# Prashant-ambati/Federated-Learning-for-Privacy-Preserving-Image-Classification

Hardware: AMD Instinct MI355X
Metric: client-images/sec/node (higher is better)
Workload: dtype f32; 1 GPU; KT: cifar10_cnn 32 clients (32/GPU), non_iid(a=0.5), 1 local epoch(s), batch 32, sgd lr 0.01, DP eps=None, FedAvg; clients=32, images_per_round=45015, batch=32, parallelism=client-packed x1 GPU

## Files before the change

### federated-learning-for-privacy-preserving-image-classification_amd/csrc/layers.hip

```cpp
#include "fh_common.h"

namespace fh {

typedef float hf32x4 __attribute__((ext_vector_type(4)));

__global__ void __launch_bounds__(256)
maxpool2_fwd_kernel(const float* __restrict__ x, int64_t x_cs, float* __restrict__ y,
                    int64_t y_cs, uint8_t* __restrict__ idx, int64_t i_cs,
                    uint8_t* __restrict__ mask, int64_t m_cs, const int32_t* __restrict__ counts,
                    int batch, int C, int H, int W, int drop_mode, float keep_prob, float scale,
                    uint64_t seed_salt, const uint64_t* __restrict__ seed_dev,
                    const float* __restrict__ in_scale, const float* __restrict__ in_shift,
                    int64_t aff_cs, int xh, int xw, int yh, int yw) {
    const uint64_t seed = seed_salt + (seed_dev ? *seed_dev : 0ull);
    const int z = blockIdx.y;
    const uint64_t prow = drop_mode == 1 ? philox_row(seed_dev, z) : 0ull;
    const int cnt = counts ? counts[z] : batch;
    const int OH = H / 2, OW = W / 2;
    const uint32_t per_img = (uint32_t)(C * OH * OW);
    const uint32_t total = (uint32_t)cnt * per_img;
    const float* xb = x + z * x_cs;
    for (uint32_t e = blockIdx.x * blockDim.x + threadIdx.x; e < total;
         e += gridDim.x * blockDim.x) {
        const uint32_t t = e / (uint32_t)OW;
        const int ow = (int)(e - t * (uint32_t)OW);
        const uint32_t plane = t / (uint32_t)OH;
        const int oh = (int)(t - plane * (uint32_t)OH);
        const float* p = xb + (int64_t)plane * xh * xw + (2 * oh) * xw + 2 * ow;
        float v0 = p[0], v1 = p[1], v2 = p[xw], v3 = p[xw + 1];
        if (in_scale) {
            const int c = (int)(plane % C);
            const float s = in_scale[z * aff_cs + c], t = in_shift[z * aff_cs + c];
            v0 = fmaxf(v0 * s + t, 0.f);
            v1 = fmaxf(v1 * s + t, 0.f);
            v2 = fmaxf(v2 * s + t, 0.f);
            v3 = fmaxf(v3 * s + t, 0.f);
        }
        float m = v0;
        int a = 0;
        if (v1 > m) { m = v1; a = 1; }
        if (v2 > m) { m = v2; a = 2; }
        if (v3 > m) { m = v3; a = 3; }
        idx[z * i_cs + e] = (uint8_t)a;
        if (drop_mode) {
            uint8_t keep;
            if (drop_mode == 1) {
                const uint4 r = Philox::gen(seed, prow, (uint64_t)e);
                keep = u01(r.x) <= keep_prob ? 1 : 0;
                mask[z * m_cs + e] = keep;
            } else {
                keep = mask[z * m_cs + e];
            }
            m = keep ? m * scale : 0.f;
        }
        y[z * y_cs + (int64_t)plane * yh * yw + oh * yw + ow] = m;
    }
}

__global__ void __launch_bounds__(256)
maxpool2_bwd_kernel(const float* __restrict__ dy, int64_t dy_cs, const uint8_t* __restrict__ idx,
                    int64_t i_cs, const uint8_t* __restrict__ mask, int64_t m_cs,
                    const float* __restrict__ xin, int64_t x_cs, float* __restrict__ dx,
                    int64_t dx_cs, const int32_t* __restrict__ counts, int batch, int C, int H,
                    int W, float scale, int gh, int gw, int xh, int xw,
                    const float* __restrict__ yin, int64_t yin_cs) {
    const int z = blockIdx.y;
    const int cnt = counts ? counts[z] : batch;
    const int OH = H / 2, OW = W / 2;
    const uint32_t total = (uint32_t)cnt * (uint32_t)(C * OH * OW);
    for (uint32_t e = blockIdx.x * blockDim.x + threadIdx.x; e < total;
         e += gridDim.x * blockDim.x) {
        const uint32_t t = e / (uint32_t)OW;
        const int ow = (int)(e - t * (uint32_t)OW);
        const uint32_t pl = t / (uint32_t)OH;
        const int oh = (int)(t - pl * (uint32_t)OH);
        const int64_t plane = pl;
        float g = dy[z * dy_cs + plane * gh * gw + oh * gw + ow];
        if (mask) g = mask[z * m_cs + e] ? g * scale : 0.f;
        const int a = idx[z * i_cs + e];
        const int64_t base = plane * xh * xw + (2 * oh) * xw + 2 * ow;
        const int64_t off[4] = {0, 1, xw, xw + 1};
        if (xin && !(xin[z * x_cs + base + off[a]] > 0.f)) g = 0.f;
        if (yin && !(yin[z * yin_cs + plane * gh * gw + oh * gw + ow] > 0.f)) g = 0.f;
        float* d = dx + z * dx_cs + base;
#pragma unroll
        for (int q = 0; q < 4; ++q) d[off[q]] = (q == a) ? g : 0.f;
    }
}

__global__ void __launch_bounds__(256)
dropout_fwd_kernel(const float* __restrict__ x, int64_t x_cs, float* __restrict__ y, int64_t y_cs,
                   uint8_t* __restrict__ mask, int64_t m_cs, const int32_t* __restrict__ counts,
                   int batch, int64_t per_img, int drop_mode, float keep_prob, float scale,
                   uint64_t seed_salt, const uint64_t* __restrict__ seed_dev) {
    const uint64_t seed = seed_salt + (seed_dev ? *seed_dev : 0ull);
    const int z = blockIdx.y;
    const uint64_t prow = drop_mode == 1 ? philox_row(seed_dev, z) : 0ull;
    const int cnt = counts ? counts[z] : batch;
    const int64_t total = cnt * per_img;
    for (int64_t e = blockIdx.x * (int64_t)blockDim.x + threadIdx.x; e < total;
         e += (int64_t)gridDim.x * blockDim.x) {
        uint8_t keep;
        if (drop_mode == 1) {
            const uint4 r = Philox::gen(seed, prow, (uint64_t)e);
            keep = u01(r.x) <= keep_prob ? 1 : 0;
            mask[z * m_cs + e] = keep;
        } else {
            keep = mask[z * m_cs + e];
        }
        const float v = x[z * x_cs + e];
        y[z * y_cs + e] = keep ? v * scale : 0.f;
    }
}

__global__ void __launch_bounds__(256)
dropout_bwd_kernel(const float* __restrict__ dy, int64_t dy_cs, const uint8_t* __restrict__ mask,
                   int64_t m_cs, const float* __restrict__ relu_out, int64_t r_cs,
                   float* __restrict__ dx, int64_t dx_cs, const int32_t* __restrict__ counts,
                   int batch, int64_t per_img, float scale) {
    const int z = blockIdx.y;
    const int cnt = counts ? counts[z] : batch;
    const int64_t total = cnt * per_img;
    for (int64_t e = blockIdx.x * (int64_t)blockDim.x + threadIdx.x; e < total;
         e += (int64_t)gridDim.x * blockDim.x) {
        float g = dy[z * dy_cs + e];
        if (mask) g = mask[z * m_cs + e] ? g * scale : 0.f;
        if (relu_out && !(relu_out[z * r_cs + e] > 0.f)) g = 0.f;
        dx[z * dx_cs + e] = g;
    }
}

__global__ void __launch_bounds__(256)
ce_kernel(const float* __restrict__ logits, int64_t l_cs, const int64_t* __restrict__ targets,
          int64_t t_cs, float* __restrict__ dlogits, int64_t d_cs, float* __restrict__ loss_out,
          double* __restrict__ acc_loss, int64_t* __restrict__ acc_correct,
          int64_t* __restrict__ acc_seen, const int32_t* __restrict__ reset,
          const int32_t* __restrict__ counts, int batch, int K) {
    __shared__ double sl[4];
    __shared__ int sc[4];
    __shared__ double li[256];
    __shared__ int ci[256];
    const int z = blockIdx.x;
    const int cnt = counts ? counts[z] : batch;
    const int lane = threadIdx.x & 63, wid = threadIdx.x >> 6;
    double lsum = 0.0;
    int corr = 0;
    const float inv_n = cnt > 0 ? 1.0f / (float)cnt : 0.f;
    if (K <= 16 && cnt <= 256) {
        const int g = threadIdx.x >> 4, l = threadIdx.x & 15;
        for (int img = g; img < cnt; img += 16) {
            const float* row = logits + z * l_cs + (int64_t)img * K;
            const int tgt = (int)targets[z * t_cs + img];
            const float v = l < K ? row[l] : -INFINITY;
            float mx = v;
            int amax = l < K ? l : K;
#pragma unroll
            for (int o = 8; o > 0; o >>= 1) {
                const float om = __shfl_xor(mx, o, 16);
                const int oa = __shfl_xor(amax, o, 16);
                if (om > mx || (om == mx && oa < amax)) { mx = om; amax = oa; }
            }
            float se = l < K ? expf(v - mx) : 0.f;
#pragma unroll
            for (int o = 8; o > 0; o >>= 1) se += __shfl_xor(se, o, 16);
            const float lse = logf(se);
            if (l == 0) {
                li[img] = (double)(-((row[tgt] - mx) - lse));
                ci[img] = amax == tgt;
            }
            if (l < K) {
                const float p = expf((v - mx) - lse);
                dlogits[z * d_cs + (int64_t)img * K + l] = (p - (l == tgt ? 1.f : 0.f)) * inv_n;
            }
        }
        __syncthreads();
        if (threadIdx.x < 4) {
            for (int img = threadIdx.x; img < cnt; img += 4) {
                lsum += li[img];
                corr += ci[img];
            }
            sl[threadIdx.x] = lsum;
            sc[threadIdx.x] = corr;
        }
        __syncthreads();
        if (threadIdx.x == 0) {
            const double tot = sl[0] + sl[1] + sl[2] + sl[3];
            const float batch_loss = cnt > 0 ? (float)(tot / (double)cnt) : 0.f;
            const bool rs = reset && reset[z];
            if (loss_out) loss_out[z] = batch_loss;
            if (acc_loss) acc_loss[z] = (rs ? 0.0 : acc_loss[z]) + (double)batch_loss;
            if (acc_correct) acc_correct[z] = (rs ? 0 : acc_correct[z]) + sc[0] + sc[1] + sc[2] + sc[3];
            if (acc_seen) acc_seen[z] = (rs ? 0 : acc_seen[z]) + cnt;
        }
        return;
    }
    for (int img = wid; img < cnt; img += 4) {
        const float* row = logits + z * l_cs + (int64_t)img * K;
        const int tgt = (int)targets[z * t_cs + img];
        float mx = -INFINITY;
        int amax = 0;
        for (int k = lane; k < K; k += 64) {
            const float v = row[k];
            if (v > mx) { mx = v; amax = k; }
        }
#pragma unroll
        for (int o = 32; o > 0; o >>= 1) {
            const float om = __shfl_xor(mx, o, 64);
            const int oa = __shfl_xor(amax, o, 64);
            if (om > mx || (om == mx && oa < amax)) { mx = om; amax = oa; }
        }
        float se = 0.f;
        for (int k = lane; k < K; k += 64) se += expf(row[k] - mx);
        se = wave_sum(se);
        const float lse = logf(se);
        if (lane == 0) {
            lsum += (double)(-((row[tgt] - mx) - lse));
            corr += (amax == tgt);
        }
        float* drow = dlogits + z * d_cs + (int64_t)img * K;
        for (int k = lane; k < K; k += 64) {
            const float p = expf((row[k] - mx) - lse);
            drow[k] = (p - (k == tgt ? 1.f : 0.f)) * inv_n;
        }
    }
    if (lane == 0) {
        sl[wid] = lsum;
        sc[wid] = corr;
    }
    __syncthreads();
    if (threadIdx.x == 0) {
        const double tot = sl[0] + sl[1] + sl[2] + sl[3];
        const float batch_loss = cnt > 0 ? (float)(tot / (double)cnt) : 0.f;
        const bool rs = reset && reset[z];
        if (loss_out) loss_out[z] = batch_loss;
        if (acc_loss) acc_loss[z] = (rs ? 0.0 : acc_loss[z]) + (double)batch_loss;
        if (acc_correct) acc_correct[z] = (rs ? 0 : acc_correct[z]) + sc[0] + sc[1] + sc[2] + sc[3];
        if (acc_seen) acc_seen[z] = (rs ? 0 : acc_seen[z]) + cnt;
    }
}

constexpr int kHeadBlocks = 4;
template <bool SMALLK>
__global__ void __launch_bounds__(256)
linear_head_ce_kernel(const float* __restrict__ x, int64_t x_cs, const float* __restrict__ w,
                      int64_t w_cs, const float* __restrict__ bias, int64_t b_cs,
                      const int64_t* __restrict__ targets, int64_t t_cs, float* __restrict__ logits,
                      int64_t l_cs, float* __restrict__ dlogits, int64_t d_cs,
                      float* __restrict__ loss_out, double* __restrict__ acc_loss,
                      int64_t* __restrict__ acc_correct, int64_t* __restrict__ acc_seen,
                      const int32_t* __restrict__ reset, float* __restrict__ dw, int64_t dw_cs,
                      float* __restrict__ db, int64_t db_cs, float* __restrict__ dx,
                      int64_t dx_cs, const uint8_t* __restrict__ mask, int64_t m_cs, float scale,
                      int relu_in, const int32_t* __restrict__ counts, int batch, int F, int K) {
    constexpr int KMAX = SMALLK ? 16 : 128;
    constexpr int FMAX = 256;
    constexpr int XS = SMALLK ? 32 * (FMAX + 1) : 1;
    constexpr int WS = SMALLK ? KMAX * (FMAX + 1) : 1;
    __shared__ float Xs[XS];
    __shared__ float Ws[WS];
    __shared__ float L[32 * KMAX];
    __shared__ float D[32 * KMAX];
    __shared__ double li[32];
    __shared__ int ci[32];
    __shared__ double sl[4];
    __shared__ int sc[4];
    constexpr int MS = SMALLK ? 32 * FMAX : 1;
    __shared__ int64_t Ts[32];
    __shared__ float Bs[KMAX];
    __shared__ uint8_t Ms[MS];
    const int z = blockIdx.y, part = blockIdx.x, tid = threadIdx.x;
    const int cnt = counts ? counts[z] : batch;
    const float* xz = x + z * x_cs;
    const float* wz = w + z * w_cs;
    const int FP = F + 1;
    const int S = gridDim.x;
    bool rs0 = false;
    double al0 = 0.0;
    int64_t ac0 = 0, as0 = 0;
    auto load_acc = [&]() {
        if (part == 0 && tid == 0) {
            rs0 = reset && reset[z];
            if (acc_loss) al0 = acc_loss[z];
            if (acc_correct) ac0 = acc_correct[z];
            if (acc_seen) as0 = acc_seen[z];
        }
    };
    const int dx_per = (cnt * F + S - 1) / S, dx_e0 = part * dx_per;
    const int dx_e1 = min(cnt * F, dx_e0 + dx_per);
    if constexpr (SMALLK) {
        const int64_t tv = tid < cnt ? targets[z * t_cs + tid] : 0;
        const float bv = (tid < K && bias) ? bias[z * b_cs + tid] : 0.f;
        const uint8_t* mz = mask + z * m_cs;
        const bool mwords = mask && dx && ((uintptr_t)mz & 3) == 0;
        constexpr int NM = 32 * FMAX / 4 / 256;
        uint32_t mw[NM];
        if (mwords) {
#pragma unroll
            for (int i = 0; i < NM; ++i) {
                const int e = tid + 256 * i;
                mw[i] = e < cnt * F / 4 ? reinterpret_cast<const uint32_t*>(mz)[e] : 0u;
            }
        }
        const bool v4 = (F & 3) == 0 && ((uintptr_t)xz & 15) == 0 && ((uintptr_t)wz & 15) == 0;
        constexpr int NX = 32 * FMAX / 4 / 256, NW = KMAX * FMAX / 4 / 256;
        const int F4 = F / 4;
        float4 xv[NX], wv[NW];
        if (v4) {
#pragma unroll
            for (int i = 0; i < NX; ++i) {
                const int e4 = tid + 256 * i;
                xv[i] = e4 < cnt * F4 ? *reinterpret_cast<const float4*>(xz + 4 * e4)
                                      : make_float4(0.f, 0.f, 0.f, 0.f);
            }
#pragma unroll
            for (int i = 0; i < NW; ++i) {
                const int e4 = tid + 256 * i;
                wv[i] = e4 < K * F4 ? *reinterpret_cast<const float4*>(wz + 4 * e4)
                                    : make_float4(0.f, 0.f, 0.f, 0.f);
            }
        }
        load_acc();
        if (tid < cnt) Ts[tid] = tv;
        if (tid < K) Bs[tid] = bv;
        if (mwords) {
#pragma unroll
            for (int i = 0; i < NM; ++i) {
                const int e = tid + 256 * i;
                if (e < cnt * F / 4) reinterpret_cast<uint32_t*>(Ms)[e] = mw[i];
            }
        } else if (mask && dx) {
            for (int e = tid; e < cnt * F; e += 256) Ms[e] = mz[e];
        }
        if (v4) {
#pragma unroll
            for (int i = 0; i < NX; ++i) {
                const int e4 = tid + 256 * i;
                if (e4 < cnt * F4) {
                    const int b = e4 / F4, f = 4 * (e4 - b * F4);
                    float* d = Xs + b * FP + f;
                    d[0] = xv[i].x; d[1] = xv[i].y; d[2] = xv[i].z; d[3] = xv[i].w;
                }
            }
#pragma unroll
            for (int i = 0; i < NW; ++i) {
                const int e4 = tid + 256 * i;
                if (e4 < K * F4) {
                    const int k = e4 / F4, f = 4 * (e4 - k * F4);
                    float* d = Ws + k * FP + f;
                    d[0] = wv[i].x; d[1] = wv[i].y; d[2] = wv[i].z; d[3] = wv[i].w;
                }
            }
        } else {
            for (int e = tid; e < cnt * F; e += 256) {
                const int b = e / F;
                Xs[b * FP + (e - b * F)] = xz[e];
            }
            for (int e = tid; e < K * F; e += 256) {
                const int k = e / F;
                Ws[k * FP + (e - k * F)] = wz[e];
            }
        }
        __syncthreads();
    } else {
        load_acc();
    }
    auto X = [&](int b, int f) -> float { return SMALLK ? Xs[b * FP + f] : xz[(int64_t)b * F + f]; };
    auto Wt = [&](int k, int f) -> float { return SMALLK ? Ws[k * FP + f] : wz[(int64_t)k * F + f]; };
    const int lane = tid & 63, wid = tid >> 6;
    if constexpr (SMALLK) {
        const int mn = lane & 15, kk = lane >> 4, t = wid & 1, fh = wid >> 1, Fh = F >> 1;
        const int ia = t * 16 + mn;
        const bool arow = ia < cnt, bcol = mn < K;
        const float* xa = Xs + ia * FP + fh * Fh + kk;
        const float* wb = Ws + mn * FP + fh * Fh + kk;
        constexpr int NQ = FMAX / 8;
        float xr[NQ], wr[NQ];
#pragma unroll
        for (int u = 0; u < NQ; ++u) {
            const float xv = xa[4 * u], wv2 = wb[4 * u];
            xr[u] = arow ? xv : 0.f;
            wr[u] = bcol ? wv2 : 0.f;
        }
        hf32x4 acc = {0.f, 0.f, 0.f, 0.f};
#pragma unroll
        for (int u = 0; u < NQ; ++u)
            if (4 * u < Fh) acc = __builtin_amdgcn_mfma_f32_16x16x4f32(xr[u], wr[u], acc, 0, 0, 0);
        float* lp = fh ? D : L;
#pragma unroll
        for (int r = 0; r < 4; ++r) lp[(t * 16 + 4 * kk + r) * 16 + mn] = acc[r];
        __syncthreads();
        float lv[2];
#pragma unroll
        for (int u = 0; u < 2; ++u) {
            const int o = tid + 256 * u;
            const int img = o / K, k = o - img * K;
            lv[u] = o < cnt * K ? L[img * 16 + k] + D[img * 16 + k] : 0.f;
        }
        __syncthreads();
#pragma unroll
        for (int u = 0; u < 2; ++u) {
            const int o = tid + 256 * u;
            if (o < cnt * K) L[o] = bias ? lv[u] + Bs[o - (o / K) * K] : lv[u];
        }
    } else {
        for (int o = tid; o < cnt * K; o += 256) {
            const int img = o / K, k = o - img * K;
            float a0 = 0.f, a1 = 0.f, a2 = 0.f, a3 = 0.f;
            for (int f = 0; f < F; f += 4) {
                a0 = fmaf(X(img, f), Wt(k, f), a0);
                a1 = fmaf(X(img, f + 1), Wt(k, f + 1), a1);
                a2 = fmaf(X(img, f + 2), Wt(k, f + 2), a2);
                a3 = fmaf(X(img, f + 3), Wt(k, f + 3), a3);
            }
            const float acc = (a0 + a1) + (a2 + a3);
            L[img * K + k] = bias ? acc + bias[z * b_cs + k] : acc;
        }
    }
    __syncthreads();
    const float inv_n = cnt > 0 ? 1.0f / (float)cnt : 0.f;
    double lsum = 0.0;
    int corr = 0;
    if (K <= 16) {
        const int g = tid >> 4, l = tid & 15;
        float v[2], mx[2], se[2];
        int amax[2], tgt[2];
#pragma unroll
        for (int u = 0; u < 2; ++u) {
            const int img = g + 16 * u;
            tgt[u] = img < cnt ? (SMALLK ? (int)Ts[img] : (int)targets[z * t_cs + img]) : 0;
            v[u] = l < K ? L[img * K + l] : -INFINITY;
            mx[u] = v[u];
            amax[u] = l < K ? l : K;
        }
#pragma unroll
        for (int o = 8; o > 0; o >>= 1)
#pragma unroll
            for (int u = 0; u < 2; ++u) {
                const float om = __shfl_xor(mx[u], o, 16);
                const int oa = __shfl_xor(amax[u], o, 16);
                if (om > mx[u] || (om == mx[u] && oa < amax[u])) { mx[u] = om; amax[u] = oa; }
            }
#pragma unroll
        for (int u = 0; u < 2; ++u) se[u] = l < K ? expf(v[u] - mx[u]) : 0.f;
#pragma unroll
        for (int o = 8; o > 0; o >>= 1)
#pragma unroll
            for (int u = 0; u < 2; ++u) se[u] += __shfl_xor(se[u], o, 16);
#pragma unroll
        for (int u = 0; u < 2; ++u) {
            const int img = g + 16 * u;
            if (img >= cnt) break;
            const float lse = logf(se[u]);
            if (l == 0) {
                li[img] = (double)(-((L[img * K + tgt[u]] - mx[u]) - lse));
                ci[img] = amax[u] == tgt[u];
            }
            if (l < K) {
                const float p = expf((v[u] - mx[u]) - lse);
                D[img * K + l] = (p - (l == tgt[u] ? 1.f : 0.f)) * inv_n;
            }
        }
        __syncthreads();
        if (tid < 4) {
            double lv[8];
            int cv[8];
#pragma unroll
            for (int j = 0; j < 8; ++j) {
                lv[j] = li[tid + 4 * j];
                cv[j] = ci[tid + 4 * j];
            }
#pragma unroll
            for (int j = 0; j < 8; ++j)
                if (tid + 4 * j < cnt) {
                    lsum += lv[j];
                    corr += cv[j];
                }
            sl[tid] = lsum;
            sc[tid] = corr;
        }
    } else {
        for (int img = wid; img < cnt; img += 4) {
            const float* row = L + img * K;
            const int tgt = (int)targets[z * t_cs + img];
            float mx = -INFINITY;
            int amax = 0;
            for (int k = lane; k < K; k += 64) {
                const float v = row[k];
                if (v > mx) { mx = v; amax = k; }
            }
#pragma unroll
            for (int o = 32; o > 0; o >>= 1) {
                const float om = __shfl_xor(mx, o, 64);
                const int oa = __shfl_xor(amax, o, 64);
                if (om > mx || (om == mx && oa < amax)) { mx = om; amax = oa; }
            }
            float se = 0.f;
            for (int k = lane; k < K; k += 64) se += expf(row[k] - mx);
            se = wave_sum(se);
            const float lse = logf(se);
            if (lane == 0) {
                lsum += (double)(-((row[tgt] - mx) - lse));
                corr += (amax == tgt);
            }
            for (int k = lane; k < K; k += 64) {
                const float p = expf((row[k] - mx) - lse);
                D[img * K + k] = (p - (k == tgt ? 1.f : 0.f)) * inv_n;
            }
        }
        if (lane == 0) {
            sl[wid] = lsum;
            sc[wid] = corr;
        }
    }
    __syncthreads();
    if (part == 0) {
        if (tid == 0) {
            const double tot = sl[0] + sl[1] + sl[2] + sl[3];
            const float batch_loss = cnt > 0 ? (float)(tot / (double)cnt) : 0.f;
            if (loss_out) loss_out[z] = batch_loss;
            if (acc_loss) acc_loss[z] = (rs0 ? 0.0 : al0) + (double)batch_loss;
            if (acc_correct) acc_correct[z] = (rs0 ? 0 : ac0) + sc[0] + sc[1] + sc[2] + sc[3];
            if (acc_seen) acc_seen[z] = (rs0 ? 0 : as0) + cnt;
        }
        for (int o = tid; o < cnt * K; o += 256) {
            logits[z * l_cs + o] = L[o];
            dlogits[z * d_cs + o] = D[o];
        }
        if (SMALLK && db && wid == 0) {
            const int k = lane & 15, g = lane >> 4;
            float v = 0.f, dv[8];
#pragma unroll
            for (int j = 0; j < 8; ++j) dv[j] = D[(g + 4 * j) * K + k];
            if (k < K)
#pragma unroll
                for (int j = 0; j < 8; ++j)
                    if (g + 4 * j < cnt) v += dv[j];
            v += __shfl_xor(v, 16, 64);
            v += __shfl_xor(v, 32, 64);
            if (lane < K) db[z * db_cs + lane] = v;
        } else if (db && tid < K) {
            float v = 0.f;
            for (int b = 0; b < cnt; ++b) v += D[b * K + tid];
            db[z * db_cs + tid] = v;
        }
    }
    if (SMALLK && dw) {
        const int mn = lane & 15, kk = lane >> 4;
        for (int tt = part + S * wid; tt < F / 16; tt += 4 * S) {
            const int f0 = tt * 16;
            float dr[8], xr2[8];
#pragma unroll
            for (int q = 0; q < 8; ++q) {
                const int b = 4 * q + kk;
                const bool ok = b < cnt;
                const float dv = D[b * K + mn], xv = Xs[b * FP + f0 + mn];
                dr[q] = ok && mn < K ? dv : 0.f;
                xr2[q] = ok ? xv : 0.f;
            }
            hf32x4 acc = {0.f, 0.f, 0.f, 0.f};
#pragma unroll
            for (int q = 0; q < 8; ++q)
                if (4 * q < cnt) acc = __builtin_amdgcn_mfma_f32_16x16x4f32(dr[q], xr2[q], acc, 0, 0, 0);
#pragma unroll
            for (int r = 0; r < 4; ++r) {
                const int k = 4 * kk + r;
                if (k < K) dw[z * dw_cs + (int64_t)k * F + f0 + mn] = acc[r];
            }
        }
    } else if (dw) {
        const int per = (K * F + S - 1) / S, e0 = part * per, e1 = min(K * F, e0 + per);
        for (int e = e0 + tid; e < e1; e += 256) {
            const int k = e / F, f = e - k * F;
            float a0 = 0.f, a1 = 0.f;
            int b = 0;
            for (; b + 1 < cnt; b += 2) {
                a0 = fmaf(D[b * K + k], X(b, f), a0);
                a1 = fmaf(D[(b + 1) * K + k], X(b + 1, f), a1);
            }
            if (b < cnt) a0 = fmaf(D[b * K + k], X(b, f), a0);
            dw[z * dw_cs + e] = a0 + a1;
        }
    }
    if (SMALLK && dx) {
        const int mn = lane & 15, kk = lane >> 4;
        for (int tt = part + S * wid; tt < 2 * (F / 16); tt += 4 * S) {
            const int t = tt & 1, f0 = (tt >> 1) * 16;
            if (t * 16 >= cnt) continue;
            const int ia = t * 16 + mn;
            float dr[KMAX / 4], wr2[KMAX / 4];
#pragma unroll
            for (int q = 0; q < KMAX / 4; ++q) {
                const int k = 4 * q + kk;
                const float dv = D[ia * K + k], wv2 = Ws[k * FP + f0 + mn];
                dr[q] = k < K && ia < cnt ? dv : 0.f;
                wr2[q] = k < K ? wv2 : 0.f;
            }
            hf32x4 acc = {0.f, 0.f, 0.f, 0.f};
#pragma unroll
            for (int q = 0; q < KMAX / 4; ++q)
                if (4 * q < K) acc = __builtin_amdgcn_mfma_f32_16x16x4f32(dr[q], wr2[q], acc, 0, 0, 0);
#pragma unroll
            for (int r = 0; r < 4; ++r) {
                const int img = t * 16 + 4 * kk + r, f = f0 + mn;
                if (img < cnt) {
                    float v = acc[r];
                    if (mask) v = Ms[img * F + f] ? v * scale : 0.f;
                    if (relu_in && !(Xs[img * FP + f] > 0.f)) v = 0.f;
                    dx[z * dx_cs + (int64_t)img * F + f] = v;
                }
            }
        }
    } else if (dx) {
        const int e0 = dx_e0, e1 = dx_e1;
        for (int eb = e0 + tid; eb < e1; eb += 4 * 256) {
            uint8_t mk[4];
#pragma unroll
            for (int u = 0; u < 4; ++u) {
                const int e = eb + 256 * u;
                mk[u] = (mask && e < e1) ? mask[z * m_cs + e] : 1;
            }
#pragma unroll
            for (int u = 0; u < 4; ++u) {
                const int e = eb + 256 * u;
                if (e >= e1) break;
                const int img = e / F, f = e - img * F;
                float acc = 0.f;
                for (int k = 0; k < K; ++k) acc = fmaf(D[img * K + k], Wt(k, f), acc);
                if (mask) acc = mk[u] ? acc * scale : 0.f;
                if (relu_in && !(X(img, f) > 0.f)) acc = 0.f;
                dx[z * dx_cs + e] = acc;
            }
        }
    }
}

__global__ void __launch_bounds__(256)
eval_metrics_kernel(const float* __restrict__ logits, int64_t l_cs,
                    const int64_t* __restrict__ targets, int64_t t_cs,
                    const int32_t* __restrict__ counts, int batch, int K,
                    double* __restrict__ loss_sum, int64_t* __restrict__ correct,
                    unsigned long long* __restrict__ class_correct,
                    unsigned long long* __restrict__ class_total) {
    __shared__ double sl[4];
    __shared__ int sc[4];
    const int z = blockIdx.x;
    const int cnt = counts ? counts[z] : batch;
    const int lane = threadIdx.x & 63, wid = threadIdx.x >> 6;
    double lsum = 0.0;
    int corr = 0;
    for (int img = wid; img < cnt; img += 4) {
        const float* row = logits + z * l_cs + (int64_t)img * K;
        const int tgt = (int)targets[z * t_cs + img];
        float mx = -INFINITY;
        int amax = 0;
        for (int k = lane; k < K; k += 64) {
            const float v = row[k];
            if (v > mx) { mx = v; amax = k; }
        }
#pragma unroll
        for (int o = 32; o > 0; o >>= 1) {
            const float om = __shfl_xor(mx, o, 64);
            const int oa = __shfl_xor(amax, o, 64);
            if (om > mx || (om == mx && oa < amax)) { mx = om; amax = oa; }
        }
        float se = 0.f;
        for (int k = lane; k < K; k += 64) se += expf(row[k] - mx);
        se = wave_sum(se);
        if (lane == 0) {
            lsum += (double)(-((row[tgt] - mx) - logf(se)));
            const int hit = amax == tgt;
            corr += hit;
            if (class_total && tgt >= 0 && tgt < K) {
                atomicAdd(class_total + tgt, 1ull);
                if (hit) atomicAdd(class_correct + tgt, 1ull);
            }
        }
    }
    if (lane == 0) {
        sl[wid] = lsum;
        sc[wid] = corr;
    }
    __syncthreads();
    if (threadIdx.x == 0) {
        if (loss_sum) loss_sum[z] += sl[0] + sl[1] + sl[2] + sl[3];
        if (correct) correct[z] += sc[0] + sc[1] + sc[2] + sc[3];
    }
}

__global__ void __launch_bounds__(256)
avgpool_fwd_kernel(const float* __restrict__ x, int64_t x_cs, float* __restrict__ y, int64_t y_cs,
                   const int32_t* __restrict__ counts, int batch, int C, int HW) {
    const int z = blockIdx.y;
    const int cnt = counts ? counts[z] : batch;
    const int lane = threadIdx.x & 63;
    const int64_t planes = (int64_t)cnt * C;
    for (int64_t pl = blockIdx.x * 4 + (threadIdx.x >> 6); pl < planes; pl += gridDim.x * 4) {
        const float* b = x + z * x_cs + pl * HW;
        float s = 0.f;
        for (int p = lane; p < HW; p += 64) s += b[p];
        s = wave_sum(s);
        if (lane == 0) y[z * y_cs + pl] = s / (float)HW;
    }
}

__global__ void __launch_bounds__(256)
avgpool_bwd_kernel(const float* __restrict__ dy, int64_t dy_cs, float* __restrict__ dx,
                   int64_t dx_cs, const int32_t* __restrict__ counts, int batch, int C, int HW) {
    const int z = blockIdx.y;
    const int cnt = counts ? counts[z] : batch;
    const int64_t total = (int64_t)cnt * C * HW;
    const float inv = 1.0f / (float)HW;
    for (int64_t e = blockIdx.x * (int64_t)blockDim.x + threadIdx.x; e < total;
         e += (int64_t)gridDim.x * blockDim.x)
        dx[z * dx_cs + e] = dy[z * dy_cs + e / HW] * inv;
}

__global__ void __launch_bounds__(256)
gather_kernel(const float* __restrict__ data, const int64_t* __restrict__ labels,
              const int64_t* __restrict__ idx, int64_t idx_cs, float* __restrict__ x, int64_t x_cs,
              int64_t* __restrict__ y, int64_t y_cs, int64_t sample_elems,
              const int32_t* __restrict__ counts, int batch) {
    const int z = blockIdx.y;
    const int cnt = counts ? counts[z] : batch;
    const int64_t total = (int64_t)cnt * sample_elems;
    constexpr int U = 4;
    const int64_t G = (int64_t)gridDim.x * blockDim.x;
    for (int64_t e0 = blockIdx.x * (int64_t)blockDim.x + threadIdx.x; e0 < total; e0 += U * G) {
        int64_t bq[U], oq[U], sq[U];
        float v[U];
#pragma unroll
        for (int u = 0; u < U; ++u) {
            const int64_t e = e0 + u * G;
            bq[u] = e < total ? e / sample_elems : 0;
            oq[u] = e - bq[u] * sample_elems;
            sq[u] = e < total ? idx[z * idx_cs + bq[u]] : 0;
        }
#pragma unroll
        for (int u = 0; u < U; ++u)
            v[u] = e0 + u * G < total ? data[sq[u] * sample_elems + oq[u]] : 0.f;
#pragma unroll
        for (int u = 0; u < U; ++u) {
            const int64_t e = e0 + u * G;
            if (e >= total) break;
            x[z * x_cs + e] = v[u];
            if (oq[u] == 0 && y) y[z * y_cs + bq[u]] = labels[sq[u]];
        }
    }
}

struct NormParams {
    float mean[4];
    float stdv[4];
};

__global__ void __launch_bounds__(256)
gather_u8_kernel(const uint8_t* __restrict__ data, const int64_t* __restrict__ labels,
                 const int64_t* __restrict__ idx, int64_t idx_cs, float* __restrict__ x,
                 int64_t x_cs, int64_t* __restrict__ y, int64_t y_cs,
                 const int32_t* __restrict__ counts, int batch, int C, int H, int W,
                 NormParams np, int pad, int flip, const uchar4* __restrict__ aug_in,
                 uchar4* __restrict__ aug_out, int64_t aug_cs, uint64_t seed_salt,
                 const uint64_t* __restrict__ seed_dev) {
    const int z = blockIdx.y;
    const int cnt = counts ? counts[z] : batch;
    const uint32_t plane = (uint32_t)(H * W), per = plane * (uint32_t)C;
    const uint32_t total = (uint32_t)cnt * per;
    const uint64_t seed = seed_salt + (seed_dev ? *seed_dev : 0ull);
    const uint64_t prow = philox_row(seed_dev, z);
    constexpr int U = 4;
    const uint32_t G = gridDim.x * blockDim.x;
    const bool aug = pad > 0 || flip;
    for (uint32_t e0 = blockIdx.x * blockDim.x + threadIdx.x; e0 < total; e0 += U * G) {
        uint32_t bq[U], rq[U];
        int cq[U], sy[U], sx[U];
        int64_t sq[U];
        uchar4 aq[U];
#pragma unroll
        for (int u = 0; u < U; ++u) {
            const uint32_t e = e0 + u * G;
            const uint32_t b = e < total ? e / per : 0u;
            bq[u] = b;
            rq[u] = e - b * per;
            sq[u] = idx[z * idx_cs + b];
            aq[u] = aug_in ? aug_in[z * aug_cs + b] : make_uchar4(0, 0, 0, 0);
        }
#pragma unroll
        for (int u = 0; u < U; ++u) {
            const uint32_t e = e0 + u * G, b = bq[u], r = rq[u];
            const int c = (int)(r / plane);
            const uint32_t p = r - (uint32_t)c * plane;
            const int yy = (int)(p / (uint32_t)W), xx = (int)(p - (uint32_t)yy * (uint32_t)W);
            int ci = pad, cj = pad, fl = 0;
            if (e < total && aug) {
                if (aug_in) {
                    ci = aq[u].x; cj = aq[u].y; fl = aq[u].z;
                } else {
                    const uint4 rr = Philox::gen(seed, prow, (uint64_t)b);
                    const uint32_t span = 2u * (uint32_t)pad + 1u;
                    ci = pad > 0 ? (int)(((uint64_t)rr.x * span) >> 32) : 0;
                    cj = pad > 0 ? (int)(((uint64_t)rr.y * span) >> 32) : 0;
                    fl = flip ? (int)(rr.z >> 31) : 0;
                    if (aug_out && r == 0) aug_out[z * aug_cs + b] = make_uchar4(ci, cj, fl, 0);
                }
            }
            const int sx0 = fl ? (W - 1 - xx) : xx;
            cq[u] = c;
            sy[u] = yy + ci - pad;
            sx[u] = sx0 + cj - pad;
        }
        uint32_t ub[U];
        int64_t lq[U];
        bool inq[U];
#pragma unroll
        for (int u = 0; u < U; ++u) {
            inq[u] = e0 + u * G < total && sy[u] >= 0 && sy[u] < H && sx[u] >= 0 && sx[u] < W;
            const int64_t off = inq[u] ? ((sq[u] * H + sy[u]) * W + sx[u]) * C + cq[u] : 0;
            ub[u] = data[off];
            lq[u] = labels[sq[u]];
        }
#pragma unroll
        for (int u = 0; u < U; ++u) {
            const uint32_t e = e0 + u * G;
            if (e >= total) break;
            const float v = __fdiv_rn(inq[u] ? (float)ub[u] : 0.f, 255.f);
            x[z * x_cs + e] = __fdiv_rn(v - np.mean[cq[u]], np.stdv[cq[u]]);
            if (rq[u] == 0 && y) y[z * y_cs + bq[u]] = lq[u];
        }
    }
}

static int ew_grid(int64_t n) { return (int)std::min<int64_t>(std::max<int64_t>(ceil_div(n, 256), 1), 2048); }

}

using namespace fh;

static int maxpool2_fwd_impl(const float* x, int64_t x_cs, const float* in_scale,
                             const float* in_shift, int64_t aff_cs, float* y, int64_t y_cs,
                             uint8_t* idx, int64_t i_cs, uint8_t* mask, int64_t m_cs,
                             const int32_t* counts, int32_t nclients, int32_t batch, int32_t C,
                             int32_t H, int32_t W, int32_t drop_mode, float p_drop, uint64_t seed,
                             const uint64_t* seed_dev, void* stream, int32_t xh = 0,
                             int32_t xw = 0, int32_t yh = 0, int32_t yw = 0) {
    if (xh == 0) { xh = H; xw = W; yh = H / 2; yw = W / 2; }
    FH_REQUIRE(nclients >= 0 && batch > 0 && C > 0 && H >= 2 && W >= 2, "maxpool2_fwd: bad shape");
    FH_REQUIRE(xh >= H && xw >= W && yh >= H / 2 && yw >= W / 2, "maxpool2_fwd: plane %dx%d / "
               "%dx%d smaller than the map %dx%d", xh, xw, yh, yw, H, W);
    FH_REQUIRE((H % 2) == 0 && (W % 2) == 0, "maxpool2_fwd: odd spatial size %dx%d", H, W);
    FH_REQUIRE(drop_mode >= 0 && drop_mode <= 2 && (drop_mode == 0 || mask), "maxpool2_fwd: mask");
    FH_REQUIRE(p_drop >= 0.f && p_drop < 1.f, "maxpool2_fwd: p=%g", p_drop);
    if (nclients == 0) return FH_OK;
    FH_REQUIRE(x && y && idx, "maxpool2_fwd: null pointer");
    const float keep = 1.0f - p_drop, scale = 1.0f / keep;
    const int64_t per = (int64_t)batch * C * (H / 2) * (W / 2);
    FH_LAUNCH(maxpool2_fwd_kernel, dim3(ew_grid(per), nclients), dim3(256), 0,
                       as_stream(stream), x, x_cs, y, y_cs, idx, i_cs, mask, m_cs, counts, batch, C,
                       H, W, drop_mode, keep, scale, seed, seed_dev, in_scale, in_shift, aff_cs,
                       xh, xw, yh, yw);
    FH_LAUNCH_CHECK("maxpool2_fwd");
    return FH_OK;
}

extern "C" int fh_maxpool2_fwd(const float* x, int64_t x_cs, float* y, int64_t y_cs, uint8_t* idx,
                               int64_t i_cs, uint8_t* mask, int64_t m_cs, const int32_t* counts,
                               int32_t nclients, int32_t batch, int32_t C, int32_t H, int32_t W,
                               int32_t drop_mode, float p_drop, uint64_t seed,
                               const uint64_t* seed_dev, void* stream) {
    return maxpool2_fwd_impl(x, x_cs, nullptr, nullptr, 0, y, y_cs, idx, i_cs, mask, m_cs, counts,
                             nclients, batch, C, H, W, drop_mode, p_drop, seed, seed_dev, stream);
}

extern "C" int fh_maxpool2_fwd_bnrelu(const float* x, int64_t x_cs, const float* in_scale,
                                      const float* in_shift, int64_t aff_cs, float* y,
                                      int64_t y_cs, uint8_t* idx, int64_t i_cs, uint8_t* mask,
                                      int64_t m_cs, const int32_t* counts, int32_t nclients,
                                      int32_t batch, int32_t C, int32_t H, int32_t W,
                                      int32_t drop_mode, float p_drop, uint64_t seed,
                                      const uint64_t* seed_dev, void* stream) {
    FH_REQUIRE(in_scale && in_shift, "maxpool2_fwd_bnrelu: null scale/shift");
    return maxpool2_fwd_impl(x, x_cs, in_scale, in_shift, aff_cs, y, y_cs, idx, i_cs, mask, m_cs,
                             counts, nclients, batch, C, H, W, drop_mode, p_drop, seed, seed_dev,
                             stream);
}

static int maxpool2_bwd_impl(const float* dy, int64_t dy_cs, const uint8_t* idx, int64_t i_cs,
                             const uint8_t* mask, int64_t m_cs, float p_drop, const float* xin,
                             int64_t x_cs, float* dx, int64_t dx_cs, const int32_t* counts,
                             int32_t nclients, int32_t batch, int32_t C, int32_t H, int32_t W,
                             void* stream, int32_t gh, int32_t gw, int32_t xh, int32_t xw,
                             const float* yin = nullptr, int64_t yin_cs = 0) {
    FH_REQUIRE(nclients >= 0 && batch > 0 && C > 0 && H >= 2 && W >= 2 && !(H & 1) && !(W & 1),
               "maxpool2_bwd: bad shape");
    FH_REQUIRE(gh >= H / 2 && gw >= W / 2 && xh >= H && xw >= W, "maxpool2_bwd: plane %dx%d / "
               "%dx%d smaller than the map %dx%d", gh, gw, xh, xw, H, W);
    if (nclients == 0) return FH_OK;
    FH_REQUIRE(dy && idx && dx, "maxpool2_bwd: null pointer");
    const float scale = 1.0f / (1.0f - p_drop);
    const int64_t per = (int64_t)batch * C * (H / 2) * (W / 2);
    FH_LAUNCH(maxpool2_bwd_kernel, dim3(ew_grid(per), nclients), dim3(256), 0,
                       as_stream(stream), dy, dy_cs, idx, i_cs, mask, m_cs, xin, x_cs, dx, dx_cs,
                       counts, batch, C, H, W, scale, gh, gw, xh, xw, yin, yin_cs);
    FH_LAUNCH_CHECK("maxpool2_bwd");
    return FH_OK;
}

extern "C" int fh_maxpool2_bwd(const float* dy, int64_t dy_cs, const uint8_t* idx, int64_t i_cs,
                               const uint8_t* mask, int64_t m_cs, float p_drop, const float* xin,
                               int64_t x_cs, float* dx, int64_t dx_cs, const int32_t* counts,
                               int32_t nclients, int32_t batch, int32_t C, int32_t H, int32_t W,
                               void* stream) {
    return maxpool2_bwd_impl(dy, dy_cs, idx, i_cs, mask, m_cs, p_drop, xin, x_cs, dx, dx_cs,
                             counts, nclients, batch, C, H, W, stream, H / 2, W / 2, H, W);
}

extern "C" int fh_maxpool2_fwd_pitched(const float* x, int64_t x_cs, float* y, int64_t y_cs,
                                       uint8_t* idx, int64_t i_cs, uint8_t* mask, int64_t m_cs,
                                       const int32_t* counts, int32_t nclients, int32_t batch,
                                       int32_t C, int32_t H, int32_t W, int32_t drop_mode,
                                       float p_drop, uint64_t seed, const uint64_t* seed_dev,
                                       int32_t xh, int32_t xw, int32_t yh, int32_t yw,
                                       void* stream) {
    FH_REQUIRE(xh > 0 && xw > 0 && yh > 0 && yw > 0, "maxpool2_fwd_pitched: bad planes");
    return maxpool2_fwd_impl(x, x_cs, nullptr, nullptr, 0, y, y_cs, idx, i_cs, mask, m_cs, counts,
                             nclients, batch, C, H, W, drop_mode, p_drop, seed, seed_dev, stream,
                             xh, xw, yh, yw);
}

extern "C" int fh_maxpool2_bwd_pitched(const float* dy, int64_t dy_cs, const uint8_t* idx,
                                       int64_t i_cs, const uint8_t* mask, int64_t m_cs,
                                       float p_drop, const float* xin, int64_t x_cs, float* dx,
                                       int64_t dx_cs, const int32_t* counts, int32_t nclients,
                                       int32_t batch, int32_t C, int32_t H, int32_t W, int32_t gh,
                                       int32_t gw, int32_t xh, int32_t xw, void* stream) {
    return maxpool2_bwd_impl(dy, dy_cs, idx, i_cs, mask, m_cs, p_drop, xin, x_cs, dx, dx_cs,
                             counts, nclients, batch, C, H, W, stream, gh, gw, xh, xw);
}

extern "C" int fh_maxpool2_bwd_ymask(const float* dy, int64_t dy_cs, const uint8_t* idx,
                                     int64_t i_cs, const float* y, int64_t y_cs, float* dx,
                                     int64_t dx_cs, const int32_t* counts, int32_t nclients,
                                     int32_t batch, int32_t C, int32_t H, int32_t W, int32_t gh,
                                     int32_t gw, int32_t xh, int32_t xw, void* stream) {
    FH_REQUIRE(y || nclients == 0, "maxpool2_bwd_ymask: null pooled output");
    return maxpool2_bwd_impl(dy, dy_cs, idx, i_cs, nullptr, 0, 0.f, nullptr, 0, dx, dx_cs, counts,
                             nclients, batch, C, H, W, stream, gh, gw, xh, xw, y, y_cs);
}

extern "C" int fh_dropout_fwd(const float* x, int64_t x_cs, float* y, int64_t y_cs, uint8_t* mask,
                              int64_t m_cs, const int32_t* counts, int32_t nclients, int32_t batch,
                              int64_t per_img, int32_t drop_mode, float p_drop, uint64_t seed,
                              const uint64_t* seed_dev, void* stream) {
    FH_REQUIRE(nclients >= 0 && batch > 0 && per_img > 0, "dropout_fwd: bad shape");
    FH_REQUIRE((drop_mode == 1 || drop_mode == 2) && mask, "dropout_fwd: mask mode");
    FH_REQUIRE(p_drop >= 0.f && p_drop < 1.f, "dropout_fwd: p=%g", p_drop);
    if (nclients == 0) return FH_OK;
    FH_REQUIRE(x && y, "dropout_fwd: null pointer");
    const float keep = 1.0f - p_drop, scale = 1.0f / keep;
    FH_LAUNCH(dropout_fwd_kernel, dim3(ew_grid(batch * per_img), nclients), dim3(256), 0,
                       as_stream(stream), x, x_cs, y, y_cs, mask, m_cs, counts, batch, per_img,
                       drop_mode, keep, scale, seed, seed_dev);
    FH_LAUNCH_CHECK("dropout_fwd");
    return FH_OK;
}

extern "C" int fh_dropout_bwd(const float* dy, int64_t dy_cs, const uint8_t* mask, int64_t m_cs,
                              float p_drop, const float* relu_out, int64_t r_cs, float* dx,
                              int64_t dx_cs, const int32_t* counts, int32_t nclients,
                              int32_t batch, int64_t per_img, void* stream) {
    FH_REQUIRE(nclients >= 0 && batch > 0 && per_img > 0, "dropout_bwd: bad shape");
    if (nclients == 0) return FH_OK;
    FH_REQUIRE(dy && dx, "dropout_bwd: null pointer");
    const float scale = 1.0f / (1.0f - p_drop);
    FH_LAUNCH(dropout_bwd_kernel, dim3(ew_grid(batch * per_img), nclients), dim3(256), 0,
                       as_stream(stream), dy, dy_cs, mask, m_cs, relu_out, r_cs, dx, dx_cs, counts,
                       batch, per_img, scale);
    FH_LAUNCH_CHECK("dropout_bwd");
    return FH_OK;
}

extern "C" int fh_ce_fwd_bwd(const float* logits, int64_t l_cs, const int64_t* targets,
                             int64_t t_cs, float* dlogits, int64_t d_cs, float* loss_out,
                             double* acc_loss, int64_t* acc_correct, int64_t* acc_seen,
                             const int32_t* reset, const int32_t* counts, int32_t nclients,
                             int32_t batch, int32_t num_classes, void* stream) {
    FH_REQUIRE(nclients >= 0 && batch > 0 && num_classes > 0, "ce_fwd_bwd: bad shape");
    if (nclients == 0) return FH_OK;
    FH_REQUIRE(logits && targets && dlogits, "ce_fwd_bwd: null pointer");
    FH_LAUNCH(ce_kernel, dim3(nclients), dim3(256), 0, as_stream(stream), logits, l_cs,
                       targets, t_cs, dlogits, d_cs, loss_out, acc_loss, acc_correct, acc_seen,
                       reset, counts, batch, num_classes);
    FH_LAUNCH_CHECK("ce_fwd_bwd");
    return FH_OK;
}

extern "C" int fh_linear_head_ce(const float* x, int64_t x_cs, const float* w, int64_t w_cs,
                                 const float* bias, int64_t b_cs, const int64_t* targets,
                                 int64_t t_cs, float* logits, int64_t l_cs, float* dlogits,
                                 int64_t d_cs, float* loss_out, double* acc_loss,
                                 int64_t* acc_correct, int64_t* acc_seen, const int32_t* reset,
                                 float* dw, int64_t dw_cs, float* db, int64_t db_cs, float* dx,
                                 int64_t dx_cs, const uint8_t* mask, int64_t m_cs, float p_drop,
                                 int32_t relu_in, const int32_t* counts, int32_t nclients,
                                 int32_t batch, int32_t in_f, int32_t num_classes, void* stream) {
    FH_REQUIRE(nclients >= 0 && batch > 0 && in_f > 0 && num_classes > 0, "linear_head_ce: bad shape");
    FH_REQUIRE(batch <= 32 && num_classes <= 128 && in_f % 4 == 0, "linear_head_ce: needs batch "
               "<= 32, <= 128 classes and in_f %% 4 == 0 (got %d, %d, %d)", batch, num_classes,
               in_f);
    FH_REQUIRE(p_drop >= 0.f && p_drop < 1.f, "linear_head_ce: p=%g", p_drop);
    if (nclients == 0) return FH_OK;
    FH_REQUIRE(x && w && targets && logits && dlogits && (dw || !db),
               "linear_head_ce: null pointer");
    const dim3 grid(kHeadBlocks, nclients);
    const float scale = 1.0f / (1.0f - p_drop);
    if (num_classes <= 16 && in_f <= 256 && in_f % 16 == 0)
        FH_LAUNCH(linear_head_ce_kernel<true>, grid, dim3(256), 0, as_stream(stream), x, x_cs, w,
                  w_cs, bias, b_cs, targets, t_cs, logits, l_cs, dlogits, d_cs, loss_out,
                  acc_loss, acc_correct, acc_seen, reset, dw, dw_cs, db, db_cs, dx, dx_cs, mask,
                  m_cs, scale, relu_in, counts, batch, in_f, num_classes);
    else
        FH_LAUNCH(linear_head_ce_kernel<false>, grid, dim3(256), 0, as_stream(stream), x, x_cs, w,
                  w_cs, bias, b_cs, targets, t_cs, logits, l_cs, dlogits, d_cs, loss_out,
                  acc_loss, acc_correct, acc_seen, reset, dw, dw_cs, db, db_cs, dx, dx_cs, mask,
                  m_cs, scale, relu_in, counts, batch, in_f, num_classes);
    FH_LAUNCH_CHECK("linear_head_ce");
    return FH_OK;
}

extern "C" int fh_eval_metrics(const float* logits, int64_t l_cs, const int64_t* targets,
                               int64_t t_cs, const int32_t* counts, int32_t nclients,
                               int32_t batch, int32_t num_classes, double* loss_sum,
                               int64_t* correct, int64_t* class_correct, int64_t* class_total,
                               void* stream) {
    FH_REQUIRE(nclients >= 0 && batch > 0 && num_classes > 0, "eval_metrics: bad shape");
    if (nclients == 0) return FH_OK;
    FH_REQUIRE(logits && targets, "eval_metrics: null pointer");
    FH_REQUIRE((class_correct == nullptr) == (class_total == nullptr),
               "eval_metrics: class_correct and class_total go together");
    FH_LAUNCH(eval_metrics_kernel, dim3(nclients), dim3(256), 0, as_stream(stream),
                       logits, l_cs, targets, t_cs, counts, batch, num_classes, loss_sum, correct,
                       reinterpret_cast<unsigned long long*>(class_correct),
                       reinterpret_cast<unsigned long long*>(class_total));
    FH_LAUNCH_CHECK("eval_metrics");
    return FH_OK;
}

extern "C" int fh_avgpool_fwd(const float* x, int64_t x_cs, float* y, int64_t y_cs,
                              const int32_t* counts, int32_t nclients, int32_t batch, int32_t C,
                              int32_t HW, void* stream) {
    FH_REQUIRE(nclients >= 0 && batch > 0 && C > 0 && HW > 0, "avgpool_fwd: bad shape");
    if (nclients == 0) return FH_OK;
    FH_REQUIRE(x && y, "avgpool_fwd: null pointer");
    const int64_t planes = (int64_t)batch * C;
    FH_LAUNCH(avgpool_fwd_kernel, dim3(ew_grid(planes * 64), nclients), dim3(256), 0,
                       as_stream(stream), x, x_cs, y, y_cs, counts, batch, C, HW);
    FH_LAUNCH_CHECK("avgpool_fwd");
    return FH_OK;
}

extern "C" int fh_avgpool_bwd(const float* dy, int64_t dy_cs, float* dx, int64_t dx_cs,
                              const int32_t* counts, int32_t nclients, int32_t batch, int32_t C,
                              int32_t HW, void* stream) {
    FH_REQUIRE(nclients >= 0 && batch > 0 && C > 0 && HW > 0, "avgpool_bwd: bad shape");
    if (nclients == 0) return FH_OK;
    FH_REQUIRE(dy && dx, "avgpool_bwd: null pointer");
    FH_LAUNCH(avgpool_bwd_kernel, dim3(ew_grid((int64_t)batch * C * HW), nclients),
                       dim3(256), 0, as_stream(stream), dy, dy_cs, dx, dx_cs, counts, batch, C, HW);
    FH_LAUNCH_CHECK("avgpool_bwd");
    return FH_OK;
}

extern "C" int fh_gather_batch(const float* data, const int64_t* labels, const int64_t* idx,
                               int64_t idx_cs, float* x, int64_t x_cs, int64_t* y, int64_t y_cs,
                               int64_t sample_elems, const int32_t* counts, int32_t nclients,
                               int32_t batch, void* stream) {
    FH_REQUIRE(nclients >= 0 && batch > 0 && sample_elems > 0, "gather_batch: bad shape");
    if (nclients == 0) return FH_OK;
    FH_REQUIRE(data && idx && x && (!y || labels), "gather_batch: null pointer");
    FH_LAUNCH(gather_kernel, dim3(ew_grid(batch * sample_elems), nclients), dim3(256), 0,
                       as_stream(stream), data, labels, idx, idx_cs, x, x_cs, y, y_cs, sample_elems,
                       counts, batch);
    FH_LAUNCH_CHECK("gather_batch");
    return FH_OK;
}

extern "C" int fh_gather_u8(const uint8_t* data, const int64_t* labels, const int64_t* idx,
                            int64_t idx_cs, float* x, int64_t x_cs, int64_t* y, int64_t y_cs,
                            const int32_t* counts, int32_t nclients, int32_t batch, int32_t C,
                            int32_t H, int32_t W, const float* mean, const float* stdv,
                            int32_t pad, int32_t flip, const uint8_t* aug_in, uint8_t* aug_out,
                            int64_t aug_cs, uint64_t seed, const uint64_t* seed_dev,
                            void* stream) {
    FH_REQUIRE(nclients >= 0 && batch > 0 && C >= 1 && C <= 4 && H > 0 && W > 0,
               "gather_u8: bad shape (C must be 1..4)");
    FH_REQUIRE(pad >= 0 && pad <= 127, "gather_u8: pad out of range");
    if (nclients == 0) return FH_OK;
    FH_REQUIRE(data && idx && x && (!y || labels) && mean && stdv, "gather_u8: null pointer");
    NormParams np;
    for (int c = 0; c < 4; ++c) {
        np.mean[c] = c < C ? mean[c] : 0.f;
        np.stdv[c] = c < C ? stdv[c] : 1.f;
    }
    FH_LAUNCH(gather_u8_kernel, dim3(ew_grid((int64_t)batch * C * H * W), nclients),
                       dim3(256), 0, as_stream(stream), data, labels, idx, idx_cs, x, x_cs, y, y_cs,
                       counts, batch, C, H, W, np, pad, flip,
                       reinterpret_cast<const uchar4*>(aug_in), reinterpret_cast<uchar4*>(aug_out),
                       aug_cs, seed, seed_dev);
    FH_LAUNCH_CHECK("gather_u8");
    return FH_OK;
}
```

Baseline: 290,700 client-images/s.

## Add per-image templated gather kernel with shared-memory staging and normalization LUT

Adds a specialized gather kernel for CIFAR and MNIST shapes in which one block handles one image. The block loads the raw uint8 image into shared memory with 16-byte loads, builds a per-channel normalization lookup table so no per-element divisions are needed, and writes the output as float4 stores. It also computes the augmentation offsets once per image rather than per element. This replaces the generic strided gather and its scattered byte loads. The cost is heavier setup per block (building the LUT and a sync) and a second code path limited to specific shapes.

Result: no change. 292,100 client-images/s, median of 6 (+0.5%).

```diff
diff --git a/federated-learning-for-privacy-preserving-image-classification_amd/csrc/layers.hip b/federated-learning-for-privacy-preserving-image-classification_amd/csrc/layers.hip
--- a/federated-learning-for-privacy-preserving-image-classification_amd/csrc/layers.hip
+++ b/federated-learning-for-privacy-preserving-image-classification_amd/csrc/layers.hip
@@ -829,6 +829,85 @@
     }
 }
 
+template <int C, int H, int W>
+__global__ void __launch_bounds__(256)
+gather_u8_image_kernel(const uint8_t* __restrict__ data, const int64_t* __restrict__ labels,
+                       const int64_t* __restrict__ idx, int64_t idx_cs, float* __restrict__ x,
+                       int64_t x_cs, int64_t* __restrict__ y, int64_t y_cs,
+                       const int32_t* __restrict__ counts, int batch, NormParams np, int pad,
+                       int flip, const uchar4* __restrict__ aug_in,
+                       uchar4* __restrict__ aug_out, int64_t aug_cs, uint64_t seed_salt,
+                       const uint64_t* __restrict__ seed_dev, int x_vec) {
+    constexpr int PER = C * H * W;
+    constexpr int NV = PER / 16;
+    constexpr int W4 = W / 4;
+    constexpr int PLANE4 = H * W4;
+    constexpr int ITEMS = C * PLANE4;
+    static_assert(PER % 16 == 0 && W % 4 == 0 && NV <= 256, "gather_u8_image_kernel: shape");
+    __shared__ float lut[C * 256];
+    __shared__ uint4 img4[NV];
+    const int z = blockIdx.y, t = threadIdx.x;
+    const int b = blockIdx.x;
+    const int cnt = counts ? counts[z] : batch;
+    if (b >= cnt) return;
+    const int64_t s = idx[z * idx_cs + b];
+    const uint4 v = reinterpret_cast<const uint4*>(data + s * PER)[t < NV ? t : 0];
+    const uchar4 rec = aug_in ? aug_in[z * aug_cs + b] : make_uchar4(0, 0, 0, 0);
+    const bool lead = t == 0;
+    const int64_t lab = (lead && y) ? labels[s] : 0;
+#pragma unroll
+    for (int c = 0; c < C; ++c)
+        lut[c * 256 + t] = __fdiv_rn(__fdiv_rn((float)t, 255.f) - np.mean[c], np.stdv[c]);
+    int ci = pad, cj = pad, fl = 0;
+    if (pad > 0 || flip) {
+        if (aug_in) {
+            ci = rec.x; cj = rec.y; fl = rec.z;
+        } else {
+            const uint64_t seed = seed_salt + (seed_dev ? *seed_dev : 0ull);
+            const uint4 rr = Philox::gen(seed, philox_row(seed_dev, z), (uint64_t)b);
+            const uint32_t span = 2u * (uint32_t)pad + 1u;
+            ci = pad > 0 ? (int)(((uint64_t)rr.x * span) >> 32) : 0;
+            cj = pad > 0 ? (int)(((uint64_t)rr.y * span) >> 32) : 0;
+            fl = flip ? (int)(rr.z >> 31) : 0;
+            if (aug_out && lead) aug_out[z * aug_cs + b] = make_uchar4(ci, cj, fl, 0);
+        }
+    }
+    if (lead && y) y[z * y_cs + b] = lab;
+    if (t < NV) img4[t] = v;
+    __syncthreads();
+    const uint8_t* img = reinterpret_cast<const uint8_t*>(img4);
+    float* xo = x + z * x_cs + (int64_t)b * PER;
+    const int dy = ci - pad, dx = cj - pad;
+#pragma unroll
+    for (int k = 0; k < (ITEMS + 255) / 256; ++k) {
+        const int i = k * 256 + t;
+        if (i >= ITEMS) break;
+        const int c = i / PLANE4, p = i - c * PLANE4;
+        const int yy = p / W4, x4 = p - yy * W4;
+        const int sy = yy + dy;
+        const bool row_in = sy >= 0 && sy < H;
+        const int row = (sy < 0 ? 0 : sy >= H ? H - 1 : sy) * W;
+        bool in[4];
+        uint32_t u[4];
+        float o[4];
+#pragma unroll
+        for (int q = 0; q < 4; ++q) {
+            const int xx = x4 * 4 + q;
+            const int sx = (fl ? W - 1 - xx : xx) + dx;
+            in[q] = row_in && sx >= 0 && sx < W;
+            u[q] = img[(row + (sx < 0 ? 0 : sx >= W ? W - 1 : sx)) * C + c];
+        }
+#pragma unroll
+        for (int q = 0; q < 4; ++q) o[q] = lut[c * 256 + (in[q] ? u[q] : 0u)];
+        if (x_vec) {
+            *reinterpret_cast<float4*>(xo + 4 * i) = make_float4(o[0], o[1], o[2], o[3]);
+        } else {
+#pragma unroll
+            for (int q = 0; q < 4; ++q) xo[4 * i + q] = o[q];
+        }
+    }
+}
+
 static int ew_grid(int64_t n) { return (int)std::min<int64_t>(std::max<int64_t>(ceil_div(n, 256), 1), 2048); }
 
 }
@@ -1100,11 +1179,26 @@
         np.mean[c] = c < C ? mean[c] : 0.f;
         np.stdv[c] = c < C ? stdv[c] : 1.f;
     }
-    FH_LAUNCH(gather_u8_kernel, dim3(ew_grid((int64_t)batch * C * H * W), nclients),
-                       dim3(256), 0, as_stream(stream), data, labels, idx, idx_cs, x, x_cs, y, y_cs,
-                       counts, batch, C, H, W, np, pad, flip,
-                       reinterpret_cast<const uchar4*>(aug_in), reinterpret_cast<uchar4*>(aug_out),
-                       aug_cs, seed, seed_dev);
+    const uchar4* ain = reinterpret_cast<const uchar4*>(aug_in);
+    uchar4* aout = reinterpret_cast<uchar4*>(aug_out);
+    const bool cifar = C == 3 && H == 32 && W == 32, mnist = C == 1 && H == 28 && W == 28;
+    if ((cifar || mnist) && (uintptr_t)data % 16 == 0 &&
+        (int64_t)batch * C * H * W <= INT32_MAX) {
+        const int x_vec = (uintptr_t)x % 16 == 0 && x_cs % 4 == 0;
+        const dim3 grid(batch, nclients);
+        if (cifar)
+            FH_LAUNCH((gather_u8_image_kernel<3, 32, 32>), grid, dim3(256), 0,
+                      as_stream(stream), data, labels, idx, idx_cs, x, x_cs, y, y_cs, counts,
+                      batch, np, pad, flip, ain, aout, aug_cs, seed, seed_dev, x_vec);
+        else
+            FH_LAUNCH((gather_u8_image_kernel<1, 28, 28>), grid, dim3(256), 0,
+                      as_stream(stream), data, labels, idx, idx_cs, x, x_cs, y, y_cs, counts,
+                      batch, np, pad, flip, ain, aout, aug_cs, seed, seed_dev, x_vec);
+    } else {
+        FH_LAUNCH(gather_u8_kernel, dim3(ew_grid((int64_t)batch * C * H * W), nclients),
+                  dim3(256), 0, as_stream(stream), data, labels, idx, idx_cs, x, x_cs, y, y_cs,
+                  counts, batch, C, H, W, np, pad, flip, ain, aout, aug_cs, seed, seed_dev);
+    }
     FH_LAUNCH_CHECK("gather_u8");
     return FH_OK;
 }
```
